# geo-ant/varpro

Hardware: AMD Instinct MI355X
Metric: independent fits/sec (double-exp, m=1024, fp64) (higher is better)
Workload: dtype f64; 1 GPU; B=65536 fits/GPU, m=1024, fp64, double-exp+offset (n=3, q=2), one full LM fit per step; batch_per_gpu=65536, m=1024, batches_in_flight=2, world_size=1, parallelism=batch-sharded x1

## Files before the change

varpro_amd/csrc/vp_device.hpp:

```cpp
#pragma once
#include <hip/hip_runtime.h>
#include <stdint.h>
#include <type_traits>

#define VP_LDS __attribute__((address_space(3)))

namespace vp {

template <typename T> struct num;
template <> struct num<double> {
    static constexpr double eps = 2.220446049250313e-16;
    static constexpr double tiny = 2.2250738585072014e-308;
    static constexpr double huge = 1.7976931348623157e+308;
    static constexpr double norm2_min = 1e-290;
};
template <> struct num<float> {
    static constexpr float eps = 1.1920929e-07f;
    static constexpr float tiny = 1.17549435e-38f;
    static constexpr float huge = 3.4028235e+38f;
    static constexpr float norm2_min = 1e-30f;
};

__device__ __forceinline__ int lane_id() { return (int)(threadIdx.x & 63u); }
#ifndef VP_LANE_FRESH
#define VP_LANE_FRESH 1
#endif
__device__ __forceinline__ int lane_fresh() {
    if (!VP_LANE_FRESH) return lane_id();
// ... 368 lines not shown
```

varpro_amd/csrc/vp_fit.hpp:

```cpp
#pragma once
#include "vp_kernels.hpp"

namespace vp {

template <bool U> __device__ __forceinline__ bool pol(bool c) {
    if constexpr (U) return uni(c);
    else return c;
}
template <bool U> __device__ __forceinline__ int pol(int v) {
    if constexpr (U) return uni(v);
    else return v;
}

template <typename T, int Q, bool U = true> __device__ __forceinline__ T enorm_small(const T (&v)[Q]) {
    T s = T(0);
#pragma unroll
    for (int j = 0; j < Q; ++j) s = tfma(v[j], v[j], s);
    if (pol<U>(s > T(1e-280) && s < T(1e280))) return usqrt(s);
    T mx = T(0);
#pragma unroll
    for (int j = 0; j < Q; ++j) mx = tmax(mx, tabs(v[j]));
    if (!(mx > T(0)) || !is_finite(mx)) return (s != s) ? s : mx;
    s = T(0);
    const T inv = T(1) / mx;
// ... 911 lines not shown
    int64_t t_stride, w_stride;
    T eps;
    T ftol, xtol, gtol, stepbound;
    int patience;
    int scale_diag;
    double *trace;
    int trace_rows;
    int grid_uniform;
    int32_t *rescue;
    int rescue_slot;
};

template <typename T, int N, int Q> struct LmState {
    T x[Q], diag[Q], qtf[Q], acnorm[Q], cbest[N];
    T Rj[Q][Q];
    T fnorm, delta, par, xnorm, gnorm, pnorm, prered, dirder, objective;
    int ipvt[Q];
    int flags;
    int nfev;
};

template <typename T, class M> inline constexpr bool fit_rescue_v = M::kStatic && M::kConstLast && M::kDiagonalPairs;

template <typename T, class M, int R, int W, bool WEIGHTED, int PADM, bool RESCUE, bool SELF>
__device__ __forceinline__ bool fit_problem(const FitArgs<T, M> &a, const int64_t b, T *s_t, T *s_y, T *s_w, unsigned char *xch,
                                            LmState<T, M::N, M::Q> *st, const bool stage_grid) {
    static_assert(!(WEIGHTED && PADM != 0), "PADM is a unit-weight specialisation");
    static_assert(!RESCUE || fit_rescue_v<T, M>, "the scaled re-fit needs the constant-first sweep and diagonal pairs");
    constexpr int N = M::N, P = M::P, Q = M::Q;
    constexpr bool CF = M::kConstLast;
    constexpr int NC = CF ? N + P : N + 1 + P;
    constexpr int YC = CF ? N - 1 : N;
    constexpr int DC = YC + 1;
    constexpr int MP = 64 * R * W;
    using G = Grp<W>;
    G grp = G::make(xch);
    const int lane = grp.gl;
    const int m = a.m;

    {
        T tmp[R];
        if (stage_grid) {
            const T *tp = a.t + b * a.t_stride;
            load_rows<T, R, W>(tp, m, lane, vec_aligned<T>(tp, m), tmp);
            store_rows<T, R, W>(s_t, MP, lane, true, tmp);
        }
        if constexpr (WEIGHTED) {
            const T *wp = a.w + b * a.w_stride;
            load_rows<T, R, W>(wp, m, lane, vec_aligned<T>(wp, m), tmp);
            store_rows<T, R, W>(s_w, MP, lane, true, tmp);
        }
        const T *yp = a.yw + b * (int64_t)m;
        load_rows<T, R, W>(yp, m, lane, vec_aligned<T>(yp, m), tmp);
        store_rows<T, R, W>(s_y, MP, lane, true, tmp);
    }
    if constexpr (W > 1) {
        __syncthreads();
    } else {
        __builtin_amdgcn_wave_barrier();
        asm volatile("s_waitcnt lgkmcnt(0)" ::: "memory");
    }
    using Src = RowSource<T, R, true, WEIGHTED ? 1 : 0, 1, W, true, PADM>;
    Src src;
    src.t = s_t;
    src.w = s_w;
    src.m = m;
    src.lane = lane;
    src.vec = true;
    src.set_uniform(a.grid_uniform != 0);
    ConstReflector<T> h0;
    if constexpr (CF) h0 = make_const_reflector<T, R, Src, G>(src, grp);

    T x[Q], xt[Q], diag[Q], qtf[Q], step[Q], acnorm[Q], cbest[N];
    T Rj[Q][Q];
    int ipvt[Q];
#pragma unroll
    for (int k = 0; k < Q; ++k) {
        xt[k] = a.alpha[b * Q + k];
        x[k] = xt[k];
        diag[k] = T(1);
        qtf[k] = T(0);
        step[k] = T(0);
        acnorm[k] = T(0);
        ipvt[k] = k;
#pragma unroll
        for (int j = 0; j < Q; ++j) Rj[k][j] = T(0);
    }
// ... 78 lines not shown
        dirder = st->dirder;
        objective = st->objective;
        {
            const int fl = uni(st->flags);
            first = (fl & 1) != 0;
            first_tr = (fl & 2) != 0;
            first_update = (fl & 4) != 0;
            nfev = uni(st->nfev);
        }
    };
    for (;;) {
        park();
        asm volatile("" ::: "memory");

        T C[NC][R];
        EvalUniform<T, N> u;
        if constexpr (R >= 2) load_rows_lds<T, R, W>(s_y, lane, C[YC]);
        else load_rows<T, R, W>(s_y, MP, lane, true, C[YC]);
        VP_TICK(clk, 0);
        int ks[N];
#pragma unroll
        for (int j = 0; j < N; ++j) ks[j] = 0;
        if constexpr (RESCUE) {
            const T t_first = s_t[0], t_last = s_t[m - 1];
#pragma unroll
            for (int j = 0; j < N - 1; ++j) {
                const T rt = T(1) / xt[j];
                const T e2 = tmax(-t_first * rt, -t_last * rt) * T(1.4426950408889634);
                ks[j] = uni((e2 > T(64) && e2 < T(1100)) ? (int)e2 : 0);
            }
            evaluate_core_const_first<T, M, R, NC, Src, G, false, false, true>(a.mdl, xt, src, a.eps, grp, h0, C, u, clk, T(0), ks);
        } else if constexpr (CF) evaluate_core_const_first<T, M, R, NC, Src, G>(a.mdl, xt, src, a.eps, grp, h0, C, u, clk);
        else evaluate_core<T, M, R, NC, Src, G>(a.mdl, xt, src, a.eps, grp, C, u, clk);
        VP_TICK(clk, 3);

        asm volatile("" ::: "memory");
        unpark();

        const T fnorm1 = usqrt(u.fn2);
        bool need_jac = false;
        if (first) {
            first = false;
            nfev = 1;
            st_best = u.ok ? VP_ST_OK : VP_ST_NONFINITE;
            if (!u.ok) {
                term = VP_TERM_USER;
                break;
// ... 382 lines not shown
```

varpro_amd/csrc/vp_fit2.hpp:

```cpp
#pragma once
#include "vp_fit.hpp"

namespace vp {

template <typename T, int N, int Q> struct alignas(8) SlotRec {
    T xt[Q], x[Q], diag[Q], qtf[Q], acnorm[Q], cbest[N], cnew[N];
    T Rj[Q][Q];
    T fnorm, delta, par, xnorm, gnorm, pnorm, prered, dirder, objective;
    T fnorm1, actred, ratio;
    T qty0;
    T pre[2 * Q + 2];
    int ipvt[Q];
    int flags;
    int nfev;
    int term;
    int status;
    int prob;
    int trow;
    int pend[2];
};

#ifndef VP_FIT2_PRE
#define VP_FIT2_PRE 1
#endif
// ... 46 lines not shown

template <typename T, typename TO = T> struct SlotConsts {
    T ftol, xtol, gtol, stepbound;
    TO *alpha;
    TO *C_out;
    double *cost_out;
    int32_t *status;
    vp_report *report;
    double *trace;
    const TO *yw;
    int *queue;
    int32_t *rescue;
    int rescue_slot;
    int self_rescue;
    int64_t B;
    int trace_rows, scale_diag, max_fev, m;
    T eps;
    T pre_delta;
#ifdef VP_FIT2_CLOCKS
    long long sck[6];
#endif
};

template <typename T, int R, class Src, class G>
__device__ __forceinline__ T fill_slot_column(const T *__restrict__ yp, const int m, T *s_col, const Src &src,
                                              const ConstReflector<T> &h0, G &grp) {
    using L = Layout<R, G::W>;
    constexpr int VW = L::VW;
    const int lane = grp.gl;
    T y[R];
    load_rows<T, R, G::W>(yp, m, lane, vec_aligned<T>(yp, m), y);
    T acc = T(0);
#pragma unroll
    for (int r0 = 0; r0 < R; r0 += VW) {
        T tt[2], sc[2];
        src.get(r0, tt, sc);
#pragma unroll
        for (int e = 0; e < VW; ++e) acc = tfma(sc[e], y[r0 + e], acc);
    }
    const T d = group_sum(grp, acc);
    const T top = group_row<R>(grp, y, 0);
    const T tau = h0.g * tfma(-h0.beta, top, d);
#pragma unroll
    for (int r0 = 0; r0 < R; r0 += VW) {
        T tt[2], sc[2];
        src.get(r0, tt, sc);
#pragma unroll
        for (int e = 0; e < VW; ++e) {
            const T v = (r0 + e < VW && L::row_of(r0 + e, lane) == 0) ? h0.u : sc[e];
            y[r0 + e] = tfma(tau, v, y[r0 + e]);
        }
    }
    store_rows<T, R, G::W>(s_col, 64 * R * G::W, lane, true, y);
    return tfma(tau, h0.u, top);
}

template <typename T, int N, int Q, int R, int W, int PADM>
__device__ VP_SLOT_FN void slot_fill(VP_LDS SlotRec<T, N, Q> *rec, VP_LDS T *s_col, VP_LDS const T *s_t,
                                       VP_LDS const SlotConsts<T> *k, VP_LDS unsigned char *xch, const int prob,
                                       const T h0_beta, const T h0_u, const T h0_g) {
    using G = Grp<W>;
    G grp = G::make((unsigned char *)xch);
    if constexpr (W == 1) grp.lane = grp.gl = slot_lane();
    const int lane = grp.gl;
    if constexpr (W > 1) __syncthreads();
    if (prob < 0) {
        if (lane == 0) {
            rec->prob = -1;
            rec->term = VP_TERM_NOT_RUN;
        }
        if constexpr (W > 1) __syncthreads();
        return;
    }
    using Src = RowSource<T, R, true, 0, 1, W, true, PADM>;
    Src src;
    src.t = (const T *)s_t;
    src.w = nullptr;
    src.m = k->m;
    src.lane = lane;
    src.vec = true;
    ConstReflector<T> h0;
    h0.beta = h0_beta;
    h0.u = h0_u;
    h0.g = h0_g;
    h0.live = true;
    const T qty0 = fill_slot_column<T, R, Src, G>(k->yw + (int64_t)prob * k->m, k->m, (T *)s_col, src, h0, grp);
    if (lane == 0) {
        const T *a0 = k->alpha + (int64_t)prob * Q;
#pragma unroll
        for (int i = 0; i < Q; ++i) {
            const T v = a0[i];
            rec->xt[i] = v;
            rec->x[i] = v;
            rec->diag[i] = T(1);
            rec->qtf[i] = T(0);
            rec->acnorm[i] = T(0);
            rec->ipvt[i] = i;
// ... 7 lines not shown
        }
        rec->fnorm = rec->delta = rec->par = rec->xnorm = rec->gnorm = rec->pnorm = rec->prered = rec->dirder = T(0);
        rec->objective = T(0) / T(0);
        rec->fnorm1 = rec->actred = rec->ratio = T(0);
        rec->qty0 = qty0;
        if constexpr (VP_FIT2_PRE != 0) {
            const T pd = k->pre_delta;
#pragma unroll
            for (int i = 0; i < Q; ++i) {
                const T rti = frcp(a0[i]);
                rec->pre[2 * i] = rti;
                rec->pre[2 * i + 1] = texp(-div_refined(pd, a0[i], rti));
            }
            rec->pre[2 * Q] = rec->pre[2 * Q + 1] = T(0);
        }
        rec->flags = 1 | 2 | 4;
        rec->nfev = 0;
        rec->term = VP_TERM_NOT_RUN;
        rec->status = VP_ST_NOT_EVALUATED;
        rec->prob = prob;
        rec->trow = 0;
    }
    if constexpr (W > 1) __syncthreads();
}

template <typename T, int N, int Q, int GS, typename TO = T, bool GRAM = false>
__device__ __forceinline__ bool slot_scalar_phase_inl(VP_LDS SlotRec<T, N, Q> *recs, VP_LDS const SlotConsts<T, TO> *k, const bool act = true,
                                                      const int lane = lane_id()) {
#ifdef VP_FIT2_CLOCKS
    long long sc0_ = __builtin_amdgcn_s_memtime();
    const bool sck_on_ = blockIdx.x == 0 && (threadIdx.x >> 6) == 0;
#define VP_SCK(i)                                                                                                      \
    do {                                                                                                               \
        const long long c1_ = __builtin_amdgcn_s_memtime();                                                           \
        if (sck_on_ && lane == 0) const_cast<SlotConsts<T, TO> *>((const SlotConsts<T, TO> *)k)->sck[i] += c1_ - sc0_;   \
        sc0_ = c1_;                                                                                                    \
    } while (0)
#else
#define VP_SCK(i)
#endif
    if (!(act && lane < GS && recs[lane].prob >= 0)) return false;
    VP_LDS SlotRec<T, N, Q> *s = recs + lane;
    const T ftol = k->ftol, xtol = k->xtol, gtol = k->gtol, stepbound = k->stepbound;
    const int scale_diag = k->scale_diag, max_fev = k->max_fev, m = k->m;
    T x[Q], xt[Q], diag[Q], qtf[Q], acnorm[Q], step[Q];
    T Rj[Q][Q];
// ... 241 lines not shown
            for (int i = 0; i < N; ++i) C_out[prob * N + i] = (TO)s->cbest[i];
        }
    }
    VP_SCK(5);
    return term != 0;
}

#if VP_FIT2_SKIP_REFILL
template <typename T, int N, int Q, int GS, typename TO = T, bool GRAM = false>
__device__ VP_SLOT_FN int slot_scalar_phase(VP_LDS SlotRec<T, N, Q> *recs, VP_LDS const SlotConsts<T, TO> *k, const bool act = true) {
    const bool done = slot_scalar_phase_inl<T, N, Q, GS, TO, GRAM>(recs, k, act, slot_lane());
    return __builtin_amdgcn_ballot_w64(done) != 0 ? 1 : 0;
}
#else
template <typename T, int N, int Q, int GS, typename TO = T, bool GRAM = false>
__device__ VP_SLOT_FN void slot_scalar_phase(VP_LDS SlotRec<T, N, Q> *recs, VP_LDS const SlotConsts<T, TO> *k, const bool act = true) {
    (void)slot_scalar_phase_inl<T, N, Q, GS, TO, GRAM>(recs, k, act, slot_lane());
}
#endif

#ifndef VP_LONE_TAIL_LINKAGE
#define VP_LONE_TAIL_LINKAGE __forceinline__
#endif
template <typename T, class M, int R, int PADM>
__device__ VP_LONE_TAIL_LINKAGE void fit2_lone_tail(VP_LDS SlotRec<T, M::N, M::Q> *rec, VP_LDS const T *s_col, VP_LDS const T *s_t,
                                            VP_LDS const SlotConsts<T> *kc, const M mdl, const T eps, const int uniform,
                                            const T h0_beta, const T h0_u, const T h0_g) {
    constexpr int N = M::N, P = M::P, Q = M::Q;
    constexpr int NC = N + P, YC = N - 1, DC = YC + 1;
    using G = SlotGrp<1>;
    G grp = G::make(nullptr);
    const int lane = grp.gl;
    using Src = RowSource<T, R, true, 0, 1, 1, true, PADM>;
    Src src;
    src.t = (const T *)s_t;
    src.w = nullptr;
    src.m = kc->m;
    src.lane = lane;
    src.vec = true;
    src.set_uniform(uniform != 0);
    ConstReflector<T> h0;
    h0.beta = h0_beta;
    h0.u = h0_u;
    h0.g = h0_g;
    h0.live = true;
    const T ftol = kc->ftol, xtol = kc->xtol, gtol = kc->gtol, stepbound = kc->stepbound;
    const int scale_diag = uni(kc->scale_diag), max_fev = uni(kc->max_fev), mres = uni(kc->m);
    const int64_t prob = uni(rec->prob);
    const T qty0 = rec->qty0;
    T x[Q], xt[Q], diag[Q], qtf[Q], step[Q], acnorm[Q], cbest[N];
    T Rj[Q][Q];
    int ipvt[Q];
#pragma unroll
    for (int k = 0; k < Q; ++k) {
        xt[k] = rec->xt[k];
        step[k] = T(0);
// ... 280 lines not shown
        } else if (flagged && kc->self_rescue == 0 && kc->rescue) {
            rescue_push(kc->rescue, kc->rescue_slot, prob);
        } else {
#pragma unroll
            for (int k = 0; k < Q; ++k) alpha_out[prob * Q + k] = x[k];
        }
        if (C_out) {
#pragma unroll
            for (int k = 0; k < N; ++k) C_out[prob * N + k] = cbest[k];
        }
        rec->term = term;
    }
}

#ifndef VP_SELF_RESCUE
#define VP_SELF_RESCUE 1
#endif
template <typename T, class M, int W> inline constexpr bool fit2_self_rescue_v = VP_SELF_RESCUE && W == 1 && fit_rescue_v<T, M>;

template <typename T, class M, int R>
__device__ VP_SLOT_FN void fit2_refit_flagged(const FitArgs<T, M> *a, const int64_t b, T *s_t, T *s_y, LmState<T, M::N, M::Q> *st) {
    (void)fit_problem<T, M, R, 1, false, 0, true, false>(*a, b, s_t, s_y, nullptr, nullptr, st, false);
}

template <typename T, class M, int R, int W, int PADM, int GS, int NG, int WPS>
__global__ void __launch_bounds__(64 * W * NG, (WPS * W * NG) / 4 > 0 ? (WPS * W * NG) / 4 : 1) fit2_kernel(const Fit2Args<T, M> args) {
    static_assert(M::kConstLast && M::kDiagonalPairs, "slot kernel: multi-exponential + offset models");
    static_assert(W == 1 || NG == 1, "multi-wave groups synchronise with workgroup barriers: one group per workgroup");
    constexpr int N = M::N, P = M::P, Q = M::Q;
    constexpr int NC = N + P;
    constexpr int YC = N - 1;
    constexpr int DC = YC + 1;
    constexpr int MP = 64 * R * W;
    using Rec = SlotRec<T, N, Q>;
    extern __shared__ __attribute__((aligned(16))) unsigned char smem_raw[];
    T *s_t = reinterpret_cast<T *>(smem_raw);
    const int gi = (W == 1) ? (VP_FIT2_SCALARS ? uni((int)(threadIdx.x >> 6)) : (int)(threadIdx.x >> 6)) : 0;
    T *s_y = s_t + MP + (size_t)gi * GS * MP;
    Rec *recs_all = reinterpret_cast<Rec *>(s_t + MP + (size_t)NG * GS * MP);
    Rec *recs = recs_all + (size_t)gi * GS;
    SlotConsts<T> *kc = reinterpret_cast<SlotConsts<T> *>(recs_all + (size_t)NG * GS);
    int *s_pop = reinterpret_cast<int *>(kc + 1);
    unsigned char *s_xch = reinterpret_cast<unsigned char *>(s_pop + ((GS + 3) / 4) * 4);
    using G = SlotGrp<W>;
    G grp = G::make(s_xch);
    const int lane = grp.gl;
    const int gw = (int)blockIdx.x * NG + gi;
    auto group_sync = [&]() __attribute__((always_inline)) {
        if constexpr (W > 1) {
            __syncthreads();
        } else {
            __builtin_amdgcn_wave_barrier();
            asm volatile("s_waitcnt lgkmcnt(0)" ::: "memory");
        }
    };
    T eps_;
    int m_, uniform_;
    int64_t B_;
    {
        const FitArgs<T, M> &a = args.f;
        m_ = VP_FIT2_SCALARS ? uni(a.m) : a.m;
        eps_ = VP_FIT2_SCALARS ? slot_uni(a.eps) : a.eps;
        uniform_ = VP_FIT2_SCALARS ? uni(a.grid_uniform) : a.grid_uniform;
        B_ = VP_FIT2_SCALARS ? slot_uni((int64_t)a.B) : a.B;
        T tmp[R];
        load_rows<T, R, W>(a.t, m_, lane, vec_aligned<T>(a.t, m_), tmp);
        store_rows<T, R, W>(s_t, MP, lane, true, tmp);
        if (threadIdx.x == 0) {
            kc->ftol = a.ftol;
            kc->xtol = a.xtol;
            kc->gtol = a.gtol;
            kc->stepbound = a.stepbound;
            kc->alpha = a.alpha;
            kc->rescue = a.rescue;
            kc->rescue_slot = a.rescue_slot;
            kc->self_rescue = (fit2_self_rescue_v<T, M, W> && a.rescue != nullptr) ? 1 : 0;
            kc->C_out = a.C_out;
            kc->cost_out = a.cost_out;
            kc->status = a.status;
            kc->report = a.report;
            kc->trace = a.trace;
            kc->yw = a.yw;
            kc->queue = args.queue;
            kc->B = a.B;
            kc->trace_rows = a.trace_rows;
            kc->scale_diag = a.scale_diag;
            kc->max_fev = a.patience * (Q + 1);
            kc->m = a.m;
#ifdef VP_FIT2_CLOCKS
            for (int i = 0; i < 6; ++i) kc->sck[i] = 0;
#endif
        }
    }
    __syncthreads();
    const int m = m_;
    using Src = RowSource<T, R, true, 0, 1, W, true, PADM>;
    Src src;
    src.t = s_t;
    src.w = nullptr;
    src.m = m;
    src.lane = lane;
    src.vec = true;
    src.set_uniform(uniform_ != 0);
    const ConstReflector<T> h0 = [&]() __attribute__((always_inline)) {
        ConstReflector<T> h = make_const_reflector<T, R, Src, G>(src, grp);
        if constexpr (VP_FIT2_SCALARS != 0) {
            h.beta = slot_uni(h.beta);
            h.u = slot_uni(h.u);
            h.g = slot_uni(h.g);
        }
        return h;
    }();
    const M mdl = args.f.mdl;
    if (threadIdx.x == 0) kc->pre_delta = src.uniform ? src.delta : T(0);
    __syncthreads();

    auto fill = [&](int s, int prob) __attribute__((always_inline)) {
        slot_fill<T, N, Q, R, W, PADM>((VP_LDS Rec *)(recs + s), (VP_LDS T *)(s_y + (size_t)s * MP), (VP_LDS const T *)s_t,
                                       (VP_LDS const SlotConsts<T> *)kc, (VP_LDS unsigned char *)s_xch, prob, h0.beta, h0.u,
                                       h0.g);
        if constexpr (W > 1) grp.phase = 0;
    };

    if (lane == 0) {
#pragma nounroll
        for (int s = 0; s < GS; ++s) recs[s].pend[0] = recs[s].pend[1] = -1;
    }
    int nactive = 0;
    bool queue_dry = false;
#pragma nounroll
    for (int s = 0; s < GS; ++s) {
        const int64_t prob = (int64_t)gw * GS + s;
        const bool have = prob < B_ && h0.live;
        fill(s, have ? (int)prob : -1);
        nactive += have ? 1 : 0;
    }
    group_sync();

#ifdef VP_FIT2_CLOCKS
    long long ck[4] = {0, 0, 0, 0};
    long long c0 = __builtin_amdgcn_s_memtime();
#define VP_CK2(i)                                                                                                      \
    do {                                                                                                               \
// ... 119 lines not shown
                next = uni(next);
            }
            const bool have = (int64_t)next < B_;
            fill(s, have ? next : -1);
            if (!have) {
                nactive -= 1;
                queue_dry = true;
            }
        }
        group_sync();
        VP_CK2(2);
#ifndef VP_NO_LONE_TAIL
        if constexpr (W == 1 && GS > 1) {
            if (queue_dry && nactive == 1) break;
        }
#endif
    }
#ifndef VP_NO_LONE_TAIL
    if constexpr (W == 1 && GS > 1) {
        if (nactive == 1) {
#pragma nounroll
            for (int s = 0; s < GS; ++s) {
                if (uni(recs[s].prob) < 0) continue;
                fit2_lone_tail<T, M, R, PADM>((VP_LDS Rec *)(recs + s), (VP_LDS const T *)(s_y + (size_t)s * MP),
                                              (VP_LDS const T *)s_t, (VP_LDS const SlotConsts<T> *)kc, mdl, eps_, uniform_,
                                              h0.beta, h0.u, h0.g);
            }
        }
    }
#endif
    if constexpr (fit2_self_rescue_v<T, M, W>) {
        group_sync();
        int pend[2 * GS];
#pragma unroll
        for (int s = 0; s < GS; ++s) {
            pend[2 * s] = uni(recs[s].pend[0]);
            pend[2 * s + 1] = uni(recs[s].pend[1]);
        }
        group_sync();
        static_assert(sizeof(LmState<T, N, Q>) <= sizeof(Rec) * GS, "the parked LM state of the re-fit lives in the group's records");
#pragma nounroll
        for (int i = 0; i < 2 * GS; ++i) {
            const int pb_ = dyn_get<2 * GS>(pend, i);
            if (pb_ < 0) continue;
            fit2_refit_flagged<T, M, R>(&args.f, (int64_t)pb_, s_t, s_y, reinterpret_cast<LmState<T, N, Q> *>(recs));
        }
    }
#ifdef VP_FIT2_CLOCKS
    if (args.f.trace && blockIdx.x == 0 && threadIdx.x == 0) {
        double *tr = args.f.trace + (size_t)(args.f.trace_rows - 1) * (Q + 4);
        for (int i = 0; i < 4; ++i) tr[i] = (double)ck[i];
        double *tr2 = args.f.trace + (size_t)(args.f.trace_rows - 2) * (Q + 4);
        for (int i = 0; i < 6 && i < Q + 4; ++i) tr2[i] = (double)kc->sck[i];
    }
#endif
}

template <typename T, class M, int R, int W = 1> int launch_fit2(const LaunchParams &p) {
    if constexpr (!(M::kConstLast && M::kDiagonalPairs)) {
        return launch_fit<T, M, R, W>(p);
    } else {
        constexpr int NG = (W == 1) ? 4 : 1;
        constexpr int WPS = waves_for<T, R, M::N + M::P>();
        constexpr int BPC = (4 * WPS) / (W * NG) > 0 ? (4 * WPS) / (W * NG) : 1;
        constexpr int GS = fit2_slots<T, R, W, NG, BPC, (int)sizeof(SlotRec<T, M::N, M::Q>)>();
        const int64_t cap_groups = (int64_t)p.num_cus * BPC * NG;
        const bool small = (W == 1) ? (p.B <= 16 * cap_groups) : false;
        if (p.w || p.t_stride != 0 || !p.queue || p.fit_group == 1 || (p.fit_group != 2 && small))
// ... 13 lines not shown
        a.B = p.B;
        a.t_stride = 0;
        a.w_stride = 0;
        a.eps = (T)p.eps;
        a.ftol = (T)p.opts->ftol;
        a.xtol = (T)p.opts->xtol;
        a.gtol = (T)p.opts->gtol;
        a.stepbound = (T)p.opts->stepbound;
        a.patience = p.opts->patience;
        a.scale_diag = p.opts->scale_diag;
        a.trace = p.trace;
        a.trace_rows = p.trace_rows;
        a.grid_uniform = p.grid_uniform;
        a.rescue = p.rescue;
        a.rescue_slot = p.rescue_slot;
        if (a.B <= 0) return VP_ERR_OK;
        if (p.rescue_used && !fit2_self_rescue_v<T, M, W>) *p.rescue_used = 1;
        const int64_t cap_blocks = (int64_t)p.num_cus * BPC;
        const int64_t need_blocks = (a.B + (int64_t)GS * NG - 1) / ((int64_t)GS * NG);
        const int64_t blocks = need_blocks < cap_blocks ? need_blocks : cap_blocks;
        args.queue = p.queue;
        args.waves_total = (int)(blocks * NG * W);
        if (hipMemsetD32Async((hipDeviceptr_t)p.queue, (int)(blocks * NG * GS), 1, p.stream) != hipSuccess) return VP_ERR_HIP;
        const size_t lds = (size_t)64 * R * W * sizeof(T) * (1 + (size_t)NG * GS) + (size_t)NG * GS * sizeof(SlotRec<T, M::N, M::Q>) +
                           sizeof(SlotConsts<T>) + (size_t)((GS + 3) / 4) * 4 * sizeof(int) + (size_t)group_xch_bytes<W>() + 16;
        if (lds > (size_t)(160 * 1024) / BPC) return launch_fit<T, M, R, W>(p);
#define VP_F2(PADM_)                                                                                                   \
    hipLaunchKernelGGL((fit2_kernel<T, M, R, W, PADM_, GS, NG, WPS>), dim3((unsigned)blocks), dim3(64 * W * NG), lds,   \
                       p.stream, args)
        if (p.m == 64 * R * W) {
            record_fit(p, kFitKernelSlots, 1, false);
            VP_F2(1);
        } else if (R > 2 && p.m > 64 * (R - 2) * W) {
            record_fit(p, kFitKernelSlots, 2, false);
            VP_F2(2);
        } else {
            record_fit(p, kFitKernelSlots, 0, false);
            VP_F2(0);
        }
#undef VP_F2
        return hipGetLastError() == hipSuccess ? VP_ERR_OK : VP_ERR_HIP;
    }
}

}
```

varpro_amd/csrc/vp_model.hpp:

```cpp
#pragma once
#include "../../include/varpro_hip.h"
#include "vp_device.hpp"

#ifndef VP_BUILD_CHUNK
#define VP_BUILD_CHUNK 8
#endif

namespace vp {

template <int NEXP, bool OFFSET> struct MultiExpModel {
    static constexpr int N = NEXP + (OFFSET ? 1 : 0);
    static constexpr int Q = NEXP;
    static constexpr int P = NEXP;
    static constexpr bool kStatic = true;
    __host__ __device__ constexpr int kind(int j) const { return j < NEXP ? VP_BASIS_EXP_DECAY : VP_BASIS_CONST; }
    __host__ __device__ constexpr int param(int j, int a) const { return (j < NEXP && a == 0) ? j : -1; }
    __host__ __device__ constexpr int pair_basis(int p) const { return p; }
    __host__ __device__ constexpr int pair_arg(int) const { return 0; }
    __host__ __device__ constexpr int pair_param(int p) const { return p; }
    static constexpr bool kDiagonalPairs = true;
    static constexpr bool kConstLast = OFFSET;
    __host__ __device__ constexpr int out_index(int j) const { return j; }
};

// ... 95 lines not shown
    ps = __builtin_fma(ps, z, 8.33333333332248946124e-03);
    ps = __builtin_fma(ps, z, -1.66666666666666324348e-01);
    const double s0 = __builtin_fma(r * z, ps, r);
    double pc = -1.13596475577881948265e-11;
    pc = __builtin_fma(pc, z, 2.08757232129817482790e-09);
    pc = __builtin_fma(pc, z, -2.75573143513906633035e-07);
    pc = __builtin_fma(pc, z, 2.48015872894767294178e-05);
    pc = __builtin_fma(pc, z, -1.38888888888741095749e-03);
    pc = __builtin_fma(pc, z, 4.16666666666666019037e-02);
    const double hz = 0.5 * z;
    const double w1 = 1.0 - hz;
    const double c0 = w1 + (((1.0 - w1) - hz) + z * z * pc);
    const int q = (int)k;
    const double a = (q & 1) ? c0 : s0, b = (q & 1) ? s0 : c0;
    sn = (q & 2) ? -a : a;
    cs = ((q + 1) & 2) ? -b : b;
}
__device__ __forceinline__ void tsincos(float x, float &sn, float &cs) {
    sn = tsin(x);
    cs = tcos(x);
}

template <typename T, int R, bool PADDED = false, int WMODE = 2, int VMODE = 2, int W = 1, bool RECUR = false,
          int PADM = 0, bool UNI = false, bool TCALC = false>
struct RowSource {
    const T *t;
    const T *w;
    int m;
    int lane;
    bool vec;
    bool uniform = false;
    T delta = T(0);
    T tl[2] = {T(0), T(0)};
    using L = Layout<R, W>;
    static constexpr int kGroupWaves = W;
    static constexpr bool kRecur = RECUR && sizeof(T) == 8 && (R > L::VW);
    static constexpr bool kAlwaysUniform = kRecur && UNI;
    static constexpr bool kScaleOne = PADDED && WMODE == 0 && PADM == 1;
    __device__ __forceinline__ void set_uniform(bool flag) {
        if constexpr (kRecur) {
            uniform = flag && m >= 3;
            if (uniform) delta = (t[m - 1] - t[0]) / T(m - 1) * T(64 * W * L::VW);
            if constexpr (TCALC) {
                static_assert(PADDED && UNI && WMODE == 0 && L::VW == 2, "computed grid: unweighted, uniform");
                using V2 = typename std::conditional<sizeof(T) == 8, double2, float2>::type;
                const V2 v = (reinterpret_cast<const V2 *>(t) + lane)[0];
                tl[0] = v.x;
                tl[1] = v.y;
            }
        } else {
            uniform = false;
        }
    }
    __device__ __forceinline__ bool weighted() const {
        if constexpr (WMODE == 0) return false;
        else if constexpr (WMODE == 1) return true;
        else return w != nullptr;
    }
    __device__ __forceinline__ void get(int r0, T (&tt)[2], T (&sc)[2]) const {
        const int i = L::row_of(r0, lane);
        if constexpr (TCALC) {
#pragma unroll
            for (int e = 0; e < 2; ++e) {
                tt[e] = (r0 == 0) ? tl[e] : tfma(T(r0 / 2), delta, tl[e]);
                sc[e] = T(1);
                if constexpr (PADM != 1) {
                    const bool in = i + e < m;
                    tt[e] = in ? tt[e] : T(0);
                    sc[e] = in ? T(1) : T(0);
                }
            }
            return;
        }
        if constexpr (L::VW == 2) {
            using V2 = typename std::conditional<sizeof(T) == 8, double2, float2>::type;
            if constexpr (PADDED) {
                const V2 v = (reinterpret_cast<const V2 *>(t) + lane)[(r0 / 2) * 64 * W];
                tt[0] = v.x;
                tt[1] = v.y;
                if constexpr (WMODE == 1) {
                    const V2 u = (reinterpret_cast<const V2 *>(w) + lane)[(r0 / 2) * 64 * W];
                    sc[0] = u.x;
                    sc[1] = u.y;
// ... 18 lines not shown
                } else {
                    sc[0] = in0 ? T(1) : T(0);
                    sc[1] = in1 ? T(1) : T(0);
                }
                return;
            }
        }
#pragma unroll
        for (int e = 0; e < L::VW; ++e) {
            const bool in = (i + e) < m;
            const int ic = in ? (i + e) : 0;
            const T tv = t[ic];
            tt[e] = in ? tv : T(0);
            if (weighted()) {
                const T wv = w[ic];
                sc[e] = in ? wv : T(0);
            } else {
                sc[e] = in ? T(1) : T(0);
            }
        }
    }
};

template <typename T, class M, int R, int NC, class Src, int DOFF = M::N + 1, bool SKIP_CONST = false, bool WF = true,
          bool WD = true, int JSEL = -1, bool SHIFT = false, bool PRE = false>
__device__ __forceinline__ void build_columns(const M &mdl, const T (&alpha)[M::Q], const Src &src, T (&C)[NC][R],
                                              const int *ks = nullptr, const T *pre = nullptr) {
    constexpr int N = M::N, P = M::P, Q = M::Q;
    constexpr int VW = Layout<R>::VW;
    static_assert(!WD || JSEL >= 0 || NC >= DOFF + P, "column array too small");
    int kind[N], s0[N], s1[N];
    T p0[N], p1[N], rt[N], rt2[N];
#pragma unroll
    for (int j = 0; j < N; ++j) {
        kind[j] = mdl.kind(j);
        const int i0 = mdl.param(j, 0), i1 = mdl.param(j, 1);
        p0[j] = (i0 >= 0) ? dyn_get<Q>(alpha, i0) : T(0);
        p1[j] = (i1 >= 0) ? dyn_get<Q>(alpha, i1) : T(0);
        s0[j] = -1;
        s1[j] = -1;
#pragma unroll
        for (int p = 0; p < P; ++p) {
            if (mdl.pair_basis(p) == j) {
                if (mdl.pair_arg(p) == 0) s0[j] = p;
                else s1[j] = p;
            }
        }
        if constexpr (PRE) rt[j] = (kind[j] == VP_BASIS_EXP_DECAY) ? pre[2 * mdl.param(j, 0)] : T(0);
        else rt[j] = (kind[j] == VP_BASIS_EXP_DECAY) ? frcp(p0[j]) : T(0);
        rt2[j] = rt[j] * rt[j];
    }
    constexpr bool kRecur = Src::kRecur;
    T fu[N][VW], qq[N];
    constexpr bool kTrig = kRecur && !M::kStatic;
    T fv[kTrig ? N : 1][VW], wr[kTrig ? N : 1], wi[kTrig ? N : 1];
    bool fast = false;
    constexpr bool kBatchExp = kRecur && M::kStatic;
    if constexpr (kRecur) {
        fast = src.uniform;
        if (fast) {
            if constexpr (kBatchExp && PRE) {
                static_assert(!PRE || M::kStatic, "precomputed trial-point scalars: static (multi-exponential) models");
                T tt0[2], sc0[2];
                src.get(0, tt0, sc0);
                T ax[N * VW], ex[N * VW];
#pragma unroll
                for (int j = 0; j < N; ++j) {
                    const bool decay = kind[j] == VP_BASIS_EXP_DECAY, rate = kind[j] == VP_BASIS_EXP_RATE;
#pragma unroll
                    for (int e = 0; e < VW; ++e)
                        ax[j * VW + e] = decay ? -div_refined(tt0[e], p0[j], rt[j]) : (rate ? -p0[j] * tt0[e] : T(0));
                }
                texp_n(ax, ex);
#pragma unroll
                for (int j = 0; j < N; ++j) {
#pragma unroll
                    for (int e = 0; e < VW; ++e) fu[j][e] = ex[j * VW + e];
                    qq[j] = (kind[j] == VP_BASIS_EXP_DECAY) ? pre[2 * mdl.param(j, 0) + 1] : T(1);
                }
            } else if constexpr (kBatchExp) {
                T tt0[2], sc0[2];
                src.get(0, tt0, sc0);
                T ax[N * (VW + 1)], ex[N * (VW + 1)];
#pragma unroll
                for (int j = 0; j < N; ++j) {
                    const bool decay = kind[j] == VP_BASIS_EXP_DECAY, rate = kind[j] == VP_BASIS_EXP_RATE;
#pragma unroll
                    for (int e = 0; e < VW; ++e)
                        ax[j * (VW + 1) + e] = decay ? -div_refined(tt0[e], p0[j], rt[j]) : (rate ? -p0[j] * tt0[e] : T(0));
                    ax[j * (VW + 1) + VW] = decay ? -div_refined(src.delta, p0[j], rt[j]) : (rate ? -p0[j] * src.delta : T(0));
                }
                texp_n(ax, ex);
#pragma unroll
                for (int j = 0; j < N; ++j) {
#pragma unroll
                    for (int e = 0; e < VW; ++e) fu[j][e] = ex[j * (VW + 1) + e];
                    qq[j] = ex[j * (VW + 1) + VW];
                }
            } else {
#pragma unroll
                for (int j = 0; j < N; ++j) {
                    qq[j] = T(1);
                    if (kind[j] == VP_BASIS_EXP_DECAY) qq[j] = texp(-div_refined(src.delta, p0[j], rt[j]));
                    else if (kind[j] == VP_BASIS_EXP_RATE) qq[j] = texp(-p0[j] * src.delta);
                    if constexpr (kTrig) {
// ... 9 lines not shown
                        }
                    }
                }
            }
        }
    }
    auto rotate = [&](T &re, T &im, const T wr_, const T wi_) __attribute__((always_inline)) {
        const T a_ = re, b_ = im;
        re = tmax(tmin(tfma(a_, wr_, -(b_ * wi_)), num<T>::huge), -num<T>::huge);
        im = tmax(tmin(tfma(a_, wi_, b_ * wr_), num<T>::huge), -num<T>::huge);
    };
    auto shifted = [&](T v, int j) __attribute__((always_inline)) {
        if constexpr (SHIFT) return tldexp(v, -ks[j]);
        else return v;
    };
    auto rows = [&](auto fast_c) __attribute__((always_inline)) {
        constexpr bool FAST = decltype(fast_c)::value;
#pragma unroll
        for (int r0 = 0; r0 < R; r0 += VW) {
            if constexpr (R > VP_BUILD_CHUNK)
                if (r0 % VP_BUILD_CHUNK == 0 && r0 != 0) __builtin_amdgcn_sched_barrier(0);
            T tt[2], sc[2];
            src.get(r0, tt, sc);
#pragma unroll
            for (int j = 0; j < N; ++j) {
                if constexpr (JSEL >= 0) {
                    if (j != JSEL) continue;
                }
#pragma unroll
                for (int e = 0; e < VW; ++e) {
                    const int r = r0 + e;
                    const T t = tt[e], scl = sc[e];
                    T f, d0 = T(0), d1 = T(0);
                    if (kind[j] == VP_BASIS_CONST) {
                        if constexpr (SKIP_CONST) continue;
                        f = scl;
                    } else if (kind[j] == VP_BASIS_EXP_DECAY) {
                        if constexpr (FAST) {
                            if constexpr (kBatchExp) {
                                if (r0 != 0) fu[j][e] = Src::kScaleOne ? fu[j][e] * qq[j] : tmin(fu[j][e] * qq[j], num<T>::huge);
                            } else {
                                fu[j][e] = (r0 == 0) ? texp(-div_refined(t, p0[j], rt[j]))
                                                     : tmin(fu[j][e] * qq[j], num<T>::huge);
                            }
                            f = fu[j][e] * scl;
                        } else {
// ... 120 lines not shown
```

Measured before the change: 32.74 million fits/s.

## Read shared time grid from global memory and launch one-wave workgroups

```diff
diff --git a/varpro_amd/csrc/vp_device.hpp b/varpro_amd/csrc/vp_device.hpp
--- a/varpro_amd/csrc/vp_device.hpp
+++ b/varpro_amd/csrc/vp_device.hpp
@@ -4,6 +4,7 @@
 #include <type_traits>
 
 #define VP_LDS __attribute__((address_space(3)))
+#define VP_GLB __attribute__((address_space(1)))
 
 namespace vp {
 
diff --git a/varpro_amd/csrc/vp_fit.hpp b/varpro_amd/csrc/vp_fit.hpp
--- a/varpro_amd/csrc/vp_fit.hpp
+++ b/varpro_amd/csrc/vp_fit.hpp
@@ -957,11 +957,12 @@
 
 template <typename T, class M> inline constexpr bool fit_rescue_v = M::kStatic && M::kConstLast && M::kDiagonalPairs;
 
-template <typename T, class M, int R, int W, bool WEIGHTED, int PADM, bool RESCUE, bool SELF>
+template <typename T, class M, int R, int W, bool WEIGHTED, int PADM, bool RESCUE, bool SELF, bool GGRID = false>
 __device__ __forceinline__ bool fit_problem(const FitArgs<T, M> &a, const int64_t b, T *s_t, T *s_y, T *s_w, unsigned char *xch,
                                             LmState<T, M::N, M::Q> *st, const bool stage_grid) {
     static_assert(!(WEIGHTED && PADM != 0), "PADM is a unit-weight specialisation");
     static_assert(!RESCUE || fit_rescue_v<T, M>, "the scaled re-fit needs the constant-first sweep and diagonal pairs");
+    static_assert(!GGRID || !WEIGHTED, "global grid: unit weights");
     constexpr int N = M::N, P = M::P, Q = M::Q;
     constexpr bool CF = M::kConstLast;
     constexpr int NC = CF ? N + P : N + 1 + P;
@@ -975,7 +976,7 @@
 
     {
         T tmp[R];
-        if (stage_grid) {
+        if (!GGRID && stage_grid) {
             const T *tp = a.t + b * a.t_stride;
             load_rows<T, R, W>(tp, m, lane, vec_aligned<T>(tp, m), tmp);
             store_rows<T, R, W>(s_t, MP, lane, true, tmp);
@@ -995,9 +996,9 @@
         __builtin_amdgcn_wave_barrier();
         asm volatile("s_waitcnt lgkmcnt(0)" ::: "memory");
     }
-    using Src = RowSource<T, R, true, WEIGHTED ? 1 : 0, 1, W, true, PADM>;
+    using Src = RowSource<T, R, true, WEIGHTED ? 1 : 0, 1, W, true, PADM, false, false, GGRID>;
     Src src;
-    src.t = s_t;
+    src.t = GGRID ? a.t : s_t;
     src.w = s_w;
     src.m = m;
     src.lane = lane;
@@ -1122,7 +1123,8 @@
 #pragma unroll
         for (int j = 0; j < N; ++j) ks[j] = 0;
         if constexpr (RESCUE) {
-            const T t_first = s_t[0], t_last = s_t[m - 1];
+            const T *tq = GGRID ? a.t : s_t;
+            const T t_first = tq[0], t_last = tq[m - 1];
 #pragma unroll
             for (int j = 0; j < N - 1; ++j) {
                 const T rt = T(1) / xt[j];
diff --git a/varpro_amd/csrc/vp_fit2.hpp b/varpro_amd/csrc/vp_fit2.hpp
--- a/varpro_amd/csrc/vp_fit2.hpp
+++ b/varpro_amd/csrc/vp_fit2.hpp
@@ -92,6 +92,27 @@
 #endif
 };
 
+#ifndef VP_FIT2_WAVE_WG
+#define VP_FIT2_WAVE_WG 1
+#endif
+template <class TP> inline constexpr bool is_glb_ptr_v = false;
+template <class U> inline constexpr bool is_glb_ptr_v<VP_GLB U *> = true;
+template <typename T, class M, int R, int W, int GS, int NG, bool GRID> constexpr size_t fit2_lds_bytes() {
+    return (size_t)64 * R * W * sizeof(T) * ((GRID ? 1 : 0) + (size_t)NG * GS) + (size_t)NG * GS * sizeof(SlotRec<T, M::N, M::Q>) +
+           sizeof(SlotConsts<T>) + (size_t)((GS + 3) / 4) * 4 * sizeof(int) + (size_t)group_xch_bytes<W>() + 16;
+}
+template <typename T, class M, int R, int W, int GS, int WPS> constexpr bool fit2_wave_wg_fits() {
+    constexpr int BPC4 = (4 * WPS) / (W * 4) > 0 ? (4 * WPS) / (W * 4) : 1;
+    return W == 1 && fit2_lds_bytes<T, M, R, W, GS, 4, true>() <= (size_t)(160 * 1024) / BPC4 &&
+           fit2_lds_bytes<T, M, R, W, GS, 1, false>() <= (size_t)(160 * 1024) / (4 * WPS);
+}
+template <typename T, class M, int R, int W, int PADM, int GS, int NG, int WPS> constexpr bool fit2_global_grid() {
+    return VP_FIT2_WAVE_WG != 0 && PADM != 0 && NG == 4 && fit2_wave_wg_fits<T, M, R, W, GS, WPS>();
+}
+template <typename T, class M, int R, int W, int PADM, int GS, int NG, int WPS> constexpr int fit2_groups() {
+    return (VP_FIT2_WAVE_WG == 1 && fit2_global_grid<T, M, R, W, PADM, GS, NG, WPS>()) ? 1 : NG;
+}
+
 template <typename T, int R, class Src, class G>
 __device__ __forceinline__ T fill_slot_column(const T *__restrict__ yp, const int m, T *s_col, const Src &src,
                                               const ConstReflector<T> &h0, G &grp) {
@@ -125,8 +146,8 @@
     return tfma(tau, h0.u, top);
 }
 
-template <typename T, int N, int Q, int R, int W, int PADM>
-__device__ VP_SLOT_FN void slot_fill(VP_LDS SlotRec<T, N, Q> *rec, VP_LDS T *s_col, VP_LDS const T *s_t,
+template <typename T, int N, int Q, int R, int W, int PADM, class TP>
+__device__ __forceinline__ void slot_fill_body(VP_LDS SlotRec<T, N, Q> *rec, VP_LDS T *s_col, TP s_t,
                                        VP_LDS const SlotConsts<T> *k, VP_LDS unsigned char *xch, const int prob,
                                        const T h0_beta, const T h0_u, const T h0_g) {
     using G = Grp<W>;
@@ -142,7 +163,7 @@
         if constexpr (W > 1) __syncthreads();
         return;
     }
-    using Src = RowSource<T, R, true, 0, 1, W, true, PADM>;
+    using Src = RowSource<T, R, true, 0, 1, W, true, PADM, false, false, is_glb_ptr_v<TP>>;
     Src src;
     src.t = (const T *)s_t;
     src.w = nullptr;
@@ -196,6 +217,18 @@
         rec->trow = 0;
     }
     if constexpr (W > 1) __syncthreads();
+}
+template <typename T, int N, int Q, int R, int W, int PADM>
+__device__ VP_SLOT_FN void slot_fill(VP_LDS SlotRec<T, N, Q> *rec, VP_LDS T *s_col, VP_LDS const T *s_t,
+                                       VP_LDS const SlotConsts<T> *k, VP_LDS unsigned char *xch, const int prob,
+                                       const T h0_beta, const T h0_u, const T h0_g) {
+    slot_fill_body<T, N, Q, R, W, PADM>(rec, s_col, s_t, k, xch, prob, h0_beta, h0_u, h0_g);
+}
+template <typename T, int N, int Q, int R, int W, int PADM>
+__device__ VP_SLOT_FN void slot_fill(VP_LDS SlotRec<T, N, Q> *rec, VP_LDS T *s_col, VP_GLB const T *s_t,
+                                       VP_LDS const SlotConsts<T> *k, VP_LDS unsigned char *xch, const int prob,
+                                       const T h0_beta, const T h0_u, const T h0_g) {
+    slot_fill_body<T, N, Q, R, W, PADM>(rec, s_col, s_t, k, xch, prob, h0_beta, h0_u, h0_g);
 }
 
 template <typename T, int N, int Q, int GS, typename TO = T, bool GRAM = false>
@@ -483,8 +516,8 @@
 #ifndef VP_LONE_TAIL_LINKAGE
 #define VP_LONE_TAIL_LINKAGE __forceinline__
 #endif
-template <typename T, class M, int R, int PADM>
-__device__ VP_LONE_TAIL_LINKAGE void fit2_lone_tail(VP_LDS SlotRec<T, M::N, M::Q> *rec, VP_LDS const T *s_col, VP_LDS const T *s_t,
+template <typename T, class M, int R, int PADM, class TP>
+__device__ VP_LONE_TAIL_LINKAGE void fit2_lone_tail(VP_LDS SlotRec<T, M::N, M::Q> *rec, VP_LDS const T *s_col, TP s_t,
                                             VP_LDS const SlotConsts<T> *kc, const M mdl, const T eps, const int uniform,
                                             const T h0_beta, const T h0_u, const T h0_g) {
     constexpr int N = M::N, P = M::P, Q = M::Q;
@@ -492,7 +525,7 @@
     using G = SlotGrp<1>;
     G grp = G::make(nullptr);
     const int lane = grp.gl;
-    using Src = RowSource<T, R, true, 0, 1, 1, true, PADM>;
+    using Src = RowSource<T, R, true, 0, 1, 1, true, PADM, false, false, is_glb_ptr_v<TP>>;
     Src src;
     src.t = (const T *)s_t;
     src.w = nullptr;
@@ -819,9 +852,14 @@
 __device__ VP_SLOT_FN void fit2_refit_flagged(const FitArgs<T, M> *a, const int64_t b, T *s_t, T *s_y, LmState<T, M::N, M::Q> *st) {
     (void)fit_problem<T, M, R, 1, false, 0, true, false>(*a, b, s_t, s_y, nullptr, nullptr, st, false);
 }
+template <typename T, class M, int R>
+__device__ VP_SLOT_FN void fit2_refit_flagged_global(const FitArgs<T, M> *a, const int64_t b, T *s_y, LmState<T, M::N, M::Q> *st) {
+    (void)fit_problem<T, M, R, 1, false, 0, true, false, true>(*a, b, nullptr, s_y, nullptr, nullptr, st, false);
+}
 
 template <typename T, class M, int R, int W, int PADM, int GS, int NG, int WPS>
-__global__ void __launch_bounds__(64 * W * NG, (WPS * W * NG) / 4 > 0 ? (WPS * W * NG) / 4 : 1) fit2_kernel(const Fit2Args<T, M> args) {
+__global__ void __launch_bounds__((64 * W * fit2_groups<T, M, R, W, PADM, GS, NG, WPS>()), (WPS * W * NG) / 4 > 0 ? (WPS * W * NG) / 4 : 1)
+fit2_kernel(const Fit2Args<T, M> args) {
     static_assert(M::kConstLast && M::kDiagonalPairs, "slot kernel: multi-exponential + offset models");
     static_assert(W == 1 || NG == 1, "multi-wave groups synchronise with workgroup barriers: one group per workgroup");
     constexpr int N = M::N, P = M::P, Q = M::Q;
@@ -829,20 +867,24 @@
     constexpr int YC = N - 1;
     constexpr int DC = YC + 1;
     constexpr int MP = 64 * R * W;
+    constexpr bool GG = fit2_global_grid<T, M, R, W, PADM, GS, NG, WPS>();
+    constexpr int NGK = fit2_groups<T, M, R, W, PADM, GS, NG, WPS>();
+    constexpr bool WAVE = (W == 1 && NGK == 1);
+    constexpr int TP_ = GG ? 0 : MP;
     using Rec = SlotRec<T, N, Q>;
     extern __shared__ __attribute__((aligned(16))) unsigned char smem_raw[];
     T *s_t = reinterpret_cast<T *>(smem_raw);
     const int gi = (W == 1) ? (VP_FIT2_SCALARS ? uni((int)(threadIdx.x >> 6)) : (int)(threadIdx.x >> 6)) : 0;
-    T *s_y = s_t + MP + (size_t)gi * GS * MP;
-    Rec *recs_all = reinterpret_cast<Rec *>(s_t + MP + (size_t)NG * GS * MP);
+    T *s_y = s_t + TP_ + (size_t)gi * GS * MP;
+    Rec *recs_all = reinterpret_cast<Rec *>(s_t + TP_ + (size_t)NGK * GS * MP);
     Rec *recs = recs_all + (size_t)gi * GS;
-    SlotConsts<T> *kc = reinterpret_cast<SlotConsts<T> *>(recs_all + (size_t)NG * GS);
+    SlotConsts<T> *kc = reinterpret_cast<SlotConsts<T> *>(recs_all + (size_t)NGK * GS);
     int *s_pop = reinterpret_cast<int *>(kc + 1);
     unsigned char *s_xch = reinterpret_cast<unsigned char *>(s_pop + ((GS + 3) / 4) * 4);
     using G = SlotGrp<W>;
     G grp = G::make(s_xch);
     const int lane = grp.gl;
-    const int gw = (int)blockIdx.x * NG + gi;
+    const int gw = (int)blockIdx.x * NGK + gi;
     auto group_sync = [&]() __attribute__((always_inline)) {
         if constexpr (W > 1) {
             __syncthreads();
@@ -854,15 +896,20 @@
     T eps_;
     int m_, uniform_;
     int64_t B_;
+    VP_GLB const T *g_t = nullptr;
     {
         const FitArgs<T, M> &a = args.f;
         m_ = VP_FIT2_SCALARS ? uni(a.m) : a.m;
         eps_ = VP_FIT2_SCALARS ? slot_uni(a.eps) : a.eps;
         uniform_ = VP_FIT2_SCALARS ? uni(a.grid_uniform) : a.grid_uniform;
         B_ = VP_FIT2_SCALARS ? slot_uni((int64_t)a.B) : a.B;
-        T tmp[R];
-        load_rows<T, R, W>(a.t, m_, lane, vec_aligned<T>(a.t, m_), tmp);
-        store_rows<T, R, W>(s_t, MP, lane, true, tmp);
+        if constexpr (GG) {
+            g_t = (VP_GLB const T *)(VP_FIT2_SCALARS ? slot_uni((int64_t)(uintptr_t)a.t) : (int64_t)(uintptr_t)a.t);
+        } else {
+            T tmp[R];
+            load_rows<T, R, W>(a.t, m_, lane, vec_aligned<T>(a.t, m_), tmp);
+            store_rows<T, R, W>(s_t, MP, lane, true, tmp);
+        }
         if (threadIdx.x == 0) {
             kc->ftol = a.ftol;
             kc->xtol = a.xtol;
@@ -889,11 +936,13 @@
 #endif
         }
     }
-    __syncthreads();
+    if constexpr (WAVE) group_sync();
+    else __syncthreads();
     const int m = m_;
-    using Src = RowSource<T, R, true, 0, 1, W, true, PADM>;
+    using Src = RowSource<T, R, true, 0, 1, W, true, PADM, false, false, GG>;
     Src src;
-    src.t = s_t;
+    if constexpr (GG) src.t = (const T *)g_t;
+    else src.t = s_t;
     src.w = nullptr;
     src.m = m;
     src.lane = lane;
@@ -910,12 +959,19 @@
     }();
     const M mdl = args.f.mdl;
     if (threadIdx.x == 0) kc->pre_delta = src.uniform ? src.delta : T(0);
-    __syncthreads();
+    if constexpr (WAVE) group_sync();
+    else __syncthreads();
 
     auto fill = [&](int s, int prob) __attribute__((always_inline)) {
-        slot_fill<T, N, Q, R, W, PADM>((VP_LDS Rec *)(recs + s), (VP_LDS T *)(s_y + (size_t)s * MP), (VP_LDS const T *)s_t,
-                                       (VP_LDS const SlotConsts<T> *)kc, (VP_LDS unsigned char *)s_xch, prob, h0.beta, h0.u,
-                                       h0.g);
+        if constexpr (GG) {
+            slot_fill<T, N, Q, R, W, PADM>((VP_LDS Rec *)(recs + s), (VP_LDS T *)(s_y + (size_t)s * MP), g_t,
+                                           (VP_LDS const SlotConsts<T> *)kc, (VP_LDS unsigned char *)s_xch, prob, h0.beta, h0.u,
+                                           h0.g);
+        } else {
+            slot_fill<T, N, Q, R, W, PADM>((VP_LDS Rec *)(recs + s), (VP_LDS T *)(s_y + (size_t)s * MP), (VP_LDS const T *)s_t,
+                                           (VP_LDS const SlotConsts<T> *)kc, (VP_LDS unsigned char *)s_xch, prob, h0.beta, h0.u,
+                                           h0.g);
+        }
         if constexpr (W > 1) grp.phase = 0;
     };
 
@@ -1081,9 +1137,14 @@
 #pragma nounroll
             for (int s = 0; s < GS; ++s) {
                 if (uni(recs[s].prob) < 0) continue;
-                fit2_lone_tail<T, M, R, PADM>((VP_LDS Rec *)(recs + s), (VP_LDS const T *)(s_y + (size_t)s * MP),
-                                              (VP_LDS const T *)s_t, (VP_LDS const SlotConsts<T> *)kc, mdl, eps_, uniform_,
-                                              h0.beta, h0.u, h0.g);
+                if constexpr (GG) {
+                    fit2_lone_tail<T, M, R, PADM>((VP_LDS Rec *)(recs + s), (VP_LDS const T *)(s_y + (size_t)s * MP), g_t,
+                                                  (VP_LDS const SlotConsts<T> *)kc, mdl, eps_, uniform_, h0.beta, h0.u, h0.g);
+                } else {
+                    fit2_lone_tail<T, M, R, PADM>((VP_LDS Rec *)(recs + s), (VP_LDS const T *)(s_y + (size_t)s * MP),
+                                                  (VP_LDS const T *)s_t, (VP_LDS const SlotConsts<T> *)kc, mdl, eps_, uniform_,
+                                                  h0.beta, h0.u, h0.g);
+                }
             }
         }
     }
@@ -1102,7 +1163,8 @@
         for (int i = 0; i < 2 * GS; ++i) {
             const int pb_ = dyn_get<2 * GS>(pend, i);
             if (pb_ < 0) continue;
-            fit2_refit_flagged<T, M, R>(&args.f, (int64_t)pb_, s_t, s_y, reinterpret_cast<LmState<T, N, Q> *>(recs));
+            if constexpr (GG) fit2_refit_flagged_global<T, M, R>(&args.f, (int64_t)pb_, s_y, reinterpret_cast<LmState<T, N, Q> *>(recs));
+            else fit2_refit_flagged<T, M, R>(&args.f, (int64_t)pb_, s_t, s_y, reinterpret_cast<LmState<T, N, Q> *>(recs));
         }
     }
 #ifdef VP_FIT2_CLOCKS
@@ -1162,12 +1224,16 @@
         args.queue = p.queue;
         args.waves_total = (int)(blocks * NG * W);
         if (hipMemsetD32Async((hipDeviceptr_t)p.queue, (int)(blocks * NG * GS), 1, p.stream) != hipSuccess) return VP_ERR_HIP;
-        const size_t lds = (size_t)64 * R * W * sizeof(T) * (1 + (size_t)NG * GS) + (size_t)NG * GS * sizeof(SlotRec<T, M::N, M::Q>) +
-                           sizeof(SlotConsts<T>) + (size_t)((GS + 3) / 4) * 4 * sizeof(int) + (size_t)group_xch_bytes<W>() + 16;
+        const size_t lds = fit2_lds_bytes<T, M, R, W, GS, NG, true>();
         if (lds > (size_t)(160 * 1024) / BPC) return launch_fit<T, M, R, W>(p);
+        if (fit2_global_grid<T, M, R, W, 1, GS, NG, WPS>() && ((uintptr_t)p.t & 15u) != 0) return launch_fit<T, M, R, W>(p);
 #define VP_F2(PADM_)                                                                                                   \
-    hipLaunchKernelGGL((fit2_kernel<T, M, R, W, PADM_, GS, NG, WPS>), dim3((unsigned)blocks), dim3(64 * W * NG), lds,   \
-                       p.stream, args)
+    do {                                                                                                               \
+        constexpr int NGK = fit2_groups<T, M, R, W, PADM_, GS, NG, WPS>();                                             \
+        constexpr size_t lds_k = fit2_lds_bytes<T, M, R, W, GS, NGK, !fit2_global_grid<T, M, R, W, PADM_, GS, NG, WPS>()>(); \
+        hipLaunchKernelGGL((fit2_kernel<T, M, R, W, PADM_, GS, NG, WPS>), dim3((unsigned)(blocks * (NG / NGK))),        \
+                           dim3(64 * W * NGK), lds_k, p.stream, args);                                                 \
+    } while (0)
         if (p.m == 64 * R * W) {
             record_fit(p, kFitKernelSlots, 1, false);
             VP_F2(1);
diff --git a/varpro_amd/csrc/vp_model.hpp b/varpro_amd/csrc/vp_model.hpp
--- a/varpro_amd/csrc/vp_model.hpp
+++ b/varpro_amd/csrc/vp_model.hpp
@@ -141,7 +141,7 @@
 }
 
 template <typename T, int R, bool PADDED = false, int WMODE = 2, int VMODE = 2, int W = 1, bool RECUR = false,
-          int PADM = 0, bool UNI = false, bool TCALC = false>
+          int PADM = 0, bool UNI = false, bool TCALC = false, bool GMEM = false>
 struct RowSource {
     const T *t;
     const T *w;
@@ -156,6 +156,8 @@
     static constexpr bool kRecur = RECUR && sizeof(T) == 8 && (R > L::VW);
     static constexpr bool kAlwaysUniform = kRecur && UNI;
     static constexpr bool kScaleOne = PADDED && WMODE == 0 && PADM == 1;
+    static constexpr bool kGlobal = GMEM;
+    static_assert(!GMEM || (PADDED && WMODE == 0 && !TCALC && L::VW == 2), "global grid: the unit-weight row-pair source");
     __device__ __forceinline__ void set_uniform(bool flag) {
         if constexpr (kRecur) {
             uniform = flag && m >= 3;
@@ -178,6 +180,29 @@
     }
     __device__ __forceinline__ void get(int r0, T (&tt)[2], T (&sc)[2]) const {
         const int i = L::row_of(r0, lane);
+        if constexpr (GMEM) {
+            typedef T v2_t __attribute__((ext_vector_type(2)));
+            const uint64_t a0 = (uint64_t)(uintptr_t)t;
+            const VP_GLB char *gb = (const VP_GLB char *)(uintptr_t)(((uint64_t)(uint32_t)uni((int)(a0 >> 32)) << 32) |
+                                                                      (uint64_t)(uint32_t)uni((int)(uint32_t)a0));
+            const bool maybe_pad = (PADM == 0) || (PADM == 2 && r0 >= R - L::VW);
+            if (!maybe_pad) {
+                const VP_GLB char *pb = gb + (size_t)(r0 / 2) * 64 * W * sizeof(v2_t);
+                const v2_t v = *(const VP_GLB v2_t *)(pb + (uint32_t)lane * (uint32_t)sizeof(v2_t));
+                tt[0] = v.x;
+                tt[1] = v.y;
+                sc[0] = sc[1] = T(1);
+            } else {
+                const bool in0 = i < m, in1 = i + 1 < m;
+                const T v0 = *(const VP_GLB T *)(gb + (uint32_t)(in0 ? i : 0) * (uint32_t)sizeof(T));
+                const T v1 = *(const VP_GLB T *)(gb + (uint32_t)(in1 ? i + 1 : 0) * (uint32_t)sizeof(T));
+                tt[0] = in0 ? v0 : T(0);
+                tt[1] = in1 ? v1 : T(0);
+                sc[0] = in0 ? T(1) : T(0);
+                sc[1] = in1 ? T(1) : T(0);
+            }
+            return;
+        }
         if constexpr (TCALC) {
 #pragma unroll
             for (int e = 0; e < 2; ++e) {
@@ -242,6 +267,9 @@
     }
 };
 
+template <class Src, class = void> struct row_source_global : std::false_type {};
+template <class Src> struct row_source_global<Src, std::void_t<decltype(Src::kGlobal)>> : std::integral_constant<bool, Src::kGlobal> {};
+
 template <typename T, class M, int R, int NC, class Src, int DOFF = M::N + 1, bool SKIP_CONST = false, bool WF = true,
           bool WD = true, int JSEL = -1, bool SHIFT = false, bool PRE = false>
 __device__ __forceinline__ void build_columns(const M &mdl, const T (&alpha)[M::Q], const Src &src, T (&C)[NC][R],
@@ -271,6 +299,18 @@
         rt2[j] = rt[j] * rt[j];
     }
     constexpr bool kRecur = Src::kRecur;
+    constexpr bool kGrid = row_source_global<Src>::value;
+    T tg[kGrid ? R : 1];
+    if constexpr (kGrid) {
+#pragma unroll
+        for (int r0 = 0; r0 < R; r0 += VW) {
+            T tt[2], sc[2];
+            src.get(r0, tt, sc);
+#pragma unroll
+            for (int e = 0; e < VW; ++e) tg[r0 + e] = tt[e];
+        }
+        __builtin_amdgcn_sched_barrier(0);
+    }
     T fu[N][VW], qq[N];
     constexpr bool kTrig = kRecur && !M::kStatic;
     T fv[kTrig ? N : 1][VW], wr[kTrig ? N : 1], wi[kTrig ? N : 1];
@@ -283,6 +323,10 @@
                 static_assert(!PRE || M::kStatic, "precomputed trial-point scalars: static (multi-exponential) models");
                 T tt0[2], sc0[2];
                 src.get(0, tt0, sc0);
+                if constexpr (kGrid) {
+#pragma unroll
+                    for (int e = 0; e < VW; ++e) tt0[e] = tg[e];
+                }
                 T ax[N * VW], ex[N * VW];
 #pragma unroll
                 for (int j = 0; j < N; ++j) {
@@ -301,6 +345,10 @@
             } else if constexpr (kBatchExp) {
                 T tt0[2], sc0[2];
                 src.get(0, tt0, sc0);
+                if constexpr (kGrid) {
+#pragma unroll
+                    for (int e = 0; e < VW; ++e) tt0[e] = tg[e];
+                }
                 T ax[N * (VW + 1)], ex[N * (VW + 1)];
 #pragma unroll
                 for (int j = 0; j < N; ++j) {
@@ -356,6 +404,10 @@
                 if (r0 % VP_BUILD_CHUNK == 0 && r0 != 0) __builtin_amdgcn_sched_barrier(0);
             T tt[2], sc[2];
             src.get(r0, tt, sc);
+            if constexpr (kGrid) {
+#pragma unroll
+                for (int e = 0; e < VW; ++e) tt[e] = tg[r0 + e];
+            }
 #pragma unroll
             for (int j = 0; j < N; ++j) {
                 if constexpr (JSEL >= 0) {
```

Measured after the change: 33.90 million fits/s (median of 6 runs). 1.04x the previous value.
